# WeijingShi/Point-GNN

Hardware: AMD Instinct MI355X
Metric: KITTI-shaped frames/sec (car_auto_T3 inference: graph build + GNN, 20000 pts/frame, mean E1 602k) (higher is better)
Workload: dtype f32

## Files before the change

point-gnn_amd/csrc/edge_ws.h:

```cpp
#pragma once
#include "mlp_engine.h"
#include "ws_partition.h"

namespace pgnn {

#ifndef PGNN_WS_SCHED
#define PGNN_WS_SCHED 2
#endif

constexpr int kWsWaves = 8;
constexpr int kWsSchedInts = 2 + kWsMaxSlices * kWsMaxGroups;
constexpr int kWsStampTiles = 38;
constexpr int kWsStampStride = 8 + 4 * kWsStampTiles;

struct EdgeWsArgs {
  const float *P, *Q;
  int ldv4;
  const int32_t *edges;
  int64_t n_edges;
  const int32_t *n_dev;
  const float *wp;
  int nt;
  int relu_from;
  float *out;
  int64_t ldo;
  int num_segments;
  int sorted;
  int xcds;
  int prio;
  long long *ts;
  int32_t *sched;
  int pool_pct;
  int chunk;
  int groups;
  int tile0[kWsMaxGroups + 1];
  int wg0[kWsMaxGroups + 1];
  int balanced;
  int n_wg[kWsMaxGroups];
  short swg0[kWsMaxSlices][kWsMaxGroups + 1];
  short sbase[kWsMaxSlices][kWsMaxGroups];
  float *rows_out;
  int64_t ld_rows;
  float *h1_out;
  const int32_t *nv_dev;
};

__device__ __forceinline__ float opaque_inf() {
  float inf;
  asm("v_mov_b32 %0, 0x7f800000" : "=v"(inf));
  return inf;
}
__device__ __forceinline__ float max_nc(float a, float b, float inf) {
  return __builtin_amdgcn_fmed3f(a, b, inf);
}

typedef float v2f __attribute__((ext_vector_type(2)));
__device__ __forceinline__ v2f pk_sub(v2f a, v2f b) {
  v2f d;
  asm("v_pk_add_f32 %0, %1, %2 neg_lo:[0,1] neg_hi:[0,1]"
      : "=v"(d)
      : "v"(a), "v"(b));
  return d;
}

template <int CTRL>
__device__ __forceinline__ float dpp_mov(float x) {
  return __int_as_float(
      __builtin_amdgcn_update_dpp(0, __float_as_int(x), CTRL, 0xF, 0xF, false));
}

template <int NTG>
__device__ __forceinline__ float ws_v(const v4f (&v)[NTG], int i) {
  return i < 4 * NTG ? v[i >> 2][i & 3] : kFloatLowest;
}

template <int NTG, class ARGS>
__device__ __forceinline__ void ws_flush(const ARGS &a, const float *bias_lds,
                                         int t0, int lane, int d,
                                         const v4f (&v)[NTG], bool whole,
                                         float inf) {
  if (d < 0 || d >= a.num_segments) return;
  int zero;
  asm volatile("s_mov_b32 %0, 0" : "=s"(zero));
  const int n = (lane & 15) + zero, g = lane >> 4;
  const bool b0 = n & 1, b1 = n & 2, b2 = n & 4, b3 = n & 8;
  float A[16], B[8], C[4], D[2];
#pragma unroll
  for (int j = 0; j < 16; ++j) {
    if (2 * j < 4 * NTG) {
      const float x0 = ws_v<NTG>(v, 2 * j), x1 = ws_v<NTG>(v, 2 * j + 1);
      A[j] = max_nc(b0 ? x1 : x0, dpp_mov<0xB1>(b0 ? x0 : x1), inf);
    } else {
      A[j] = kFloatLowest;
    }
  }
#pragma unroll
  for (int k = 0; k < 8; ++k)
    B[k] = max_nc(b1 ? A[2 * k + 1] : A[2 * k],
                  dpp_mov<0x4E>(b1 ? A[2 * k] : A[2 * k + 1]), inf);
#pragma unroll
  for (int l = 0; l < 4; ++l)
    C[l] = max_nc(b2 ? B[2 * l + 1] : B[2 * l],
                  __shfl_xor(b2 ? B[2 * l] : B[2 * l + 1], 4), inf);
#pragma unroll
  for (int m = 0; m < 2; ++m)
    D[m] = max_nc(b3 ? C[2 * m + 1] : C[2 * m],
                  __shfl_xor(b3 ? C[2 * m] : C[2 * m + 1], 8), inf);
  float *orow = a.out + (int64_t)d * a.ldo + 16 * t0;
#pragma unroll
  for (int m = 0; m < 2; ++m) {
    const int i = 16 * m + n;
    if (i < 4 * NTG) {
      const int c = 16 * (i >> 2) + 4 * g + (i & 3);
      float x = D[m] + bias_lds[c];
      if (16 * t0 + c >= a.relu_from) x = x > 0.0f ? x : 0.0f;
      if (whole)
        orow[c] = x;
      else
        atomic_max_f32(orow + c, x + 0.0f);
    }
  }
}

struct WsRun {
  int cur_d;
  bool left_closed;
  bool has;
};

template <int NTG, class ARGS>
__device__ __forceinline__ void ws_epilogue(const ARGS &a, const float *bias_lds,
                                            int t0, int lane,
                                            const v4f (&acc)[NTG],
                                            v4f (&carry)[NTG], unsigned starts,
                                            int my_d, WsRun &st, bool fin,
                                            int d_after, float inf) {
  const int n = lane & 15;
  int cur_d = st.cur_d;
  bool cur_left_closed = st.left_closed, cur_has = st.has;
  int pos = 0;
  if (!(starts & 1u)) {
    const int f = starts ? __builtin_ctz(starts) : 16;
    if (f == 16) {
#pragma unroll
      for (int t = 0; t < NTG; ++t)
#pragma unroll
        for (int r = 0; r < 4; ++r)
          carry[t][r] = max_nc(carry[t][r], acc[t][r], inf);
    } else {
      const bool in_run = n < f;
#pragma unroll
      for (int t = 0; t < NTG; ++t)
#pragma unroll
        for (int r = 0; r < 4; ++r)
          carry[t][r] =
              max_nc(carry[t][r], in_run ? acc[t][r] : kFloatLowest, inf);
    }
    cur_has = true;
    pos = f;
  }
  while (pos < 16) {
    if (cur_has)
      ws_flush<NTG>(a, bias_lds, t0, lane, cur_d, carry,
                    a.sorted && cur_left_closed &&
                        (!fin || d_after != cur_d),
                    inf);
    if (fin) break;
    const unsigned rest = starts & ~((2u << pos) - 1u);
    const int nextpos = rest ? __builtin_ctz(rest) : 16;
    const bool in_run = n >= pos && n < nextpos;
#pragma unroll
    for (int t = 0; t < NTG; ++t)
#pragma unroll
      for (int r = 0; r < 4; ++r)
        carry[t][r] = in_run ? acc[t][r] : kFloatLowest;
    cur_d = __builtin_amdgcn_readlane(my_d, pos);
    cur_left_closed = true;
    cur_has = true;
    pos = nextpos;
  }
  st.cur_d = cur_d;
  st.left_closed = cur_left_closed;
  st.has = cur_has;
}

}

#include "ws_sum.h"

namespace pgnn {

template <int KQ, int NTG, bool EMIT, bool ROWS = false, class POL = WsMax>
__device__ __forceinline__ void edge_ws_body(const EdgeWsArgs &a,
                                             const v4f *__restrict__ wl, int t0,
                                             const float *bias_lds,
                                             int64_t tile_first,
                                             int64_t tile_last, int lane,
                                             long long *tsw, int &stamped,
                                             const int64_t E) {
  if (tile_first >= tile_last) return;
  const int n = lane & 15;
  const int64_t e_first = tile_first * 16;
  const int64_t e_end = tile_last * 16 < E ? tile_last * 16 : E;
  const v4f *__restrict__ P4 = reinterpret_cast<const v4f *>(a.P);
  const v4f *__restrict__ Q4 = reinterpret_cast<const v4f *>(a.Q);
  const int2 *__restrict__ e2 = reinterpret_cast<const int2 *>(a.edges);

// ... 390 lines not shown
```

point-gnn_amd/csrc/mlp_engine.h:

```cpp
#pragma once
#include "pgnn_common.h"

namespace pgnn {

#ifndef PGNN_PF4
#define PGNN_PF4 2
#endif
#ifndef PGNN_PF1
#define PGNN_PF1 4
#endif

typedef float v4f __attribute__((ext_vector_type(4)));

struct LayerDev {
  const float *wp;
  int kq;
  int nt;
  int relu_from;
};

struct ChainDev {
  int n;
  LayerDev l[PGNN_MAX_LAYERS];
};
// ... 339 lines not shown
#pragma unroll
      for (int r = 0; r < NR; ++r)
        accr[r] = __builtin_amdgcn_mfma_f32_16x16x4f32(fa_r[s], fb_r[r][s],
                                                       accr[r], 0, 0, 0);
    }
  };
#pragma unroll
  for (int st = 0; st < PF; ++st) fetch(st, a[st], b[st], ar[st], br[st]);
  for (int q = 0; q < kq; q += PF) {
#pragma unroll
    for (int st = 0; st < PF; ++st) {
      if (q + st < kq) {
        mma(a[st], b[st], ar[st], br[st], 0, 4);
        fetch(q + st + PF, a[st], b[st], ar[st], br[st]);
      }
    }
  }
}

__device__ __forceinline__ float activate(const LayerDev &L, const float *bias,
                                          int col, float x) {
  x += bias[col];
  if (col >= L.relu_from) x = x > 0.0f ? x : 0.0f;
  return x;
}

template <int NT, int NR, bool TRANSPOSED>
__device__ __forceinline__ void store_split(float *__restrict__ out, int ldo,
                                            const LayerDev &L, int t0, int wave,
                                            int lane, const v4f (&acc)[4][NT],
                                            const v4f (&accr)[NR]) {
  if (TRANSPOSED)
    store_acc_T<4, NT>(out, L, t0, wave, lane, acc);
  else
    store_acc<4, NT>(out, ldo, L, t0, wave, lane, acc);
  const float *bias = L.wp + (size_t)L.kq * L.nt * 256;
  constexpr int ROWS = 64, G = ROWS / 4, SWZ = 15;
#pragma unroll
  for (int r = 0; r < NR; ++r) {
    const int col = (t0 + 4 * NT + r) * 16 + (lane & 15);
    const int c = col - 16 * t0;
    v4f v;
#pragma unroll
    for (int i = 0; i < 4; ++i) v[i] = activate(L, bias, col, accr[r][i]);
    if (TRANSPOSED) {
      const int g = 4 * wave + (lane >> 4);
      *reinterpret_cast<v4f *>(out + c * ROWS + ((g ^ (c & SWZ)) << 2)) = v;
    } else {
      float *o = out + (16 * wave + 4 * (lane >> 4)) * ldo + c;
#pragma unroll
      for (int i = 0; i < 4; ++i) o[i * ldo] = v[i];
    }
  }
  (void)G;
}

template <int NT, int NR, bool TRANSPOSED>
__device__ __forceinline__ void layer_pass_split(const float *in, int ld_in,
                                                 float *out, int ld_out,
                                                 const LayerDev &L, int t0,
                                                 int wave, int lane) {
  v4f acc[4][NT], accr[NR];
  gemm_tile_split<NT, NR>(in, ld_in, L, t0, wave, lane, acc, accr);
  __syncthreads();
  store_split<NT, NR, TRANSPOSED>(out, ld_out, L, t0, wave, lane, acc, accr);
  __syncthreads();
}

__device__ __forceinline__ void lds_atomic_max_f32(float *addr, float v) {
  if (v >= 0.0f) {
    __hip_atomic_fetch_max((int *)addr, __float_as_int(v), __ATOMIC_RELAXED,
                           __HIP_MEMORY_SCOPE_WORKGROUP);
  } else {
    __hip_atomic_fetch_min((unsigned int *)addr, __float_as_uint(v),
                           __ATOMIC_RELAXED, __HIP_MEMORY_SCOPE_WORKGROUP);
  }
}

__device__ __forceinline__ void segfast_emit(const SegFast &sf, int col,
                                             float v) {
  if (sf.merge) v = fmaxf(v, sf.carry[col]);
  if (sf.defer) {
    sf.carry[col] = v;
  } else if (sf.whole) {
    sf.out_row[col] = v;
  } else {
    atomic_max_f32(sf.out_row + col, v + 0.0f);
  }
}

template <int NT, int NR>
__device__ __forceinline__ void layer_pass_segmax_fast_split(
    const float *in, int ld_in, const LayerDev &L, int t0, int wave, int lane,
    const SegFast &sf, float *part) {
  v4f acc[4][NT], accr[NR];
  gemm_tile_split<NT, NR>(in, ld_in, L, t0, wave, lane, acc, accr);
  const float *bias = L.wp + (size_t)L.kq * L.nt * 256;
#pragma unroll
  for (int r = 0; r < NR; ++r) {
    float v = fmaxf(fmaxf(accr[r][0], accr[r][1]),
                    fmaxf(accr[r][2], accr[r][3]));
    v = fmaxf(v, __shfl_xor(v, 16));
    v = fmaxf(v, __shfl_xor(v, 32));
    if (lane < 16) lds_atomic_max_f32(part + r * 16 + lane, v + 0.0f);
  }
#pragma unroll
  for (int j = 0; j < NT; ++j) {
    float v = acc[0][j][0];
#pragma unroll
    for (int m = 0; m < 4; ++m)
#pragma unroll
      for (int i = 0; i < 4; ++i) v = fmaxf(v, acc[m][j][i]);
    v = fmaxf(v, __shfl_xor(v, 16));
    v = fmaxf(v, __shfl_xor(v, 32));
    const int col = (t0 + wave + 4 * j) * 16 + (lane & 15);
    if (lane < 16) segfast_emit(sf, col, activate(L, bias, col, v));
  }
}

template <int NT, int NR>
__device__ __forceinline__ void segfast_finish_split(const LayerDev &L, int t0,
                                                     const SegFast &sf,
                                                     float *part) {
  if (threadIdx.x < 16 * NR) {
    const float *bias = L.wp + (size_t)L.kq * L.nt * 256;
    const int col = (t0 + 4 * NT) * 16 + threadIdx.x;
    const float v = part[threadIdx.x];
    part[threadIdx.x] = kFloatLowest;
    segfast_emit(sf, col, activate(L, bias, col, v));
  }
}

__device__ __forceinline__ bool use_split(int msub, int tiles) {
  return msub == 4 && tiles == 19;
}

template <int MSUB>
__device__ __forceinline__ bool layer_pass_segmax_fast_auto(
    const float *in, int ld_in, const LayerDev &L, int t0, int wave, int lane,
    const SegFast &sf, float *part) {
  int tiles = L.nt - t0;
  if (tiles > kMaxTilesPerPass) tiles = kMaxTilesPerPass;
  if constexpr (MSUB == 4) {
    if (use_split(MSUB, tiles)) {
      layer_pass_segmax_fast_split<4, 3>(in, ld_in, L, t0, wave, lane, sf,
                                         part);
      return true;
    }
  }
  layer_pass_segmax_fast_dispatch<MSUB>(in, ld_in, L, t0, wave, lane, sf);
  return false;
}

template <int KQ, int NT, int TBMAX = 8>
__device__ __forceinline__ void reg_layer(const LayerDev &L, int lane,
                                          const v4f (&in)[KQ], v4f (&out)[NT]) {
  int zero;
  asm volatile("s_mov_b32 %0, 0" : "=s"(zero));
  const v4f *__restrict__ wp =
      reinterpret_cast<const v4f *>(L.wp) + lane + zero;
  const float *bias = L.wp + (size_t)KQ * NT * 256 + zero;
  const int g4 = 4 * (lane >> 4) + zero;
  constexpr int TB = NT < TBMAX ? NT : TBMAX;
  static_assert(NT % TB == 0, "column tiles come in blocks");
#pragma unroll
  for (int t0 = 0; t0 < NT; t0 += TB) {
    v4f w[2][TB];
#pragma unroll
    for (int j = 0; j < TB; ++j) {
      out[t0 + j] = (v4f){0.f, 0.f, 0.f, 0.f};
      w[0][j] = wp[(size_t)(t0 + j) * 64];
    }
#pragma unroll
    for (int q = 0; q < KQ; ++q) {
      if (q + 1 < KQ) {
#pragma unroll
        for (int j = 0; j < TB; ++j)
          w[(q + 1) & 1][j] = wp[((size_t)(q + 1) * NT + t0 + j) * 64];
      }
#pragma unroll
      for (int s = 0; s < 4; ++s)
#pragma unroll
        for (int j = 0; j < TB; ++j)
          out[t0 + j] = __builtin_amdgcn_mfma_f32_16x16x4f32(
              w[q & 1][j][s], in[q][s], out[t0 + j], 0, 0, 0);
      __builtin_amdgcn_sched_barrier(0);
    }
#pragma unroll
    for (int j = 0; j < TB; ++j) {
      const int t = t0 + j;
      const v4f b = *reinterpret_cast<const v4f *>(bias + 16 * t + g4);
#pragma unroll
      for (int r = 0; r < 4; ++r) {
        float v = out[t][r] + b[r];
        if (16 * t + g4 + r >= L.relu_from) v = v > 0.0f ? v : 0.0f;
        out[t][r] = v;
      }
    }
  }
}

template <int KQ, int... NTS>
struct RegChain;

template <int KQ>
struct RegChain<KQ> {
  static __device__ __forceinline__ void run(const ChainDev &, int, int lane,
                                             const v4f (&in)[KQ],
                                             float *__restrict__ rows16,
                                             int ld) {
    float *o = rows16 + (lane & 15) * ld + 4 * (lane >> 4);
#pragma unroll
    for (int q = 0; q < KQ; ++q) *reinterpret_cast<v4f *>(o + 16 * q) = in[q];
  }
};

template <int KQ, int NT, int... REST>
struct RegChain<KQ, NT, REST...> {
  static __device__ __forceinline__ void run(const ChainDev &chain, int li,
                                             int lane, const v4f (&in)[KQ],
                                             float *__restrict__ rows16,
                                             int ld) {
    v4f out[NT];
    reg_layer<KQ, NT>(chain.l[li], lane, in, out);
    RegChain<NT, REST...>::run(chain, li + 1, lane, out, rows16, ld);
  }
};

template <int MSUB, int NT, bool TRANSPOSED, int NW = 4>
__device__ __forceinline__ void layer_pass(const float *in, int ld_in, float *out,
                                           int ld_out, const LayerDev &L, int t0,
                                           int wave, int lane, bool skip_gemm) {
  static_assert(!TRANSPOSED || NW == 4, "transposed stage is 4-wave only");
  v4f acc[MSUB][NT];
  if (!skip_gemm) {
    gemm_tile<MSUB, NT, NW>(in, ld_in, L, t0, wave, lane, acc);
  } else {
#pragma unroll
    for (int m = 0; m < MSUB; ++m)
#pragma unroll
      for (int j = 0; j < NT; ++j) acc[m][j] = (v4f){0.f, 0.f, 0.f, 0.f};
  }
  __syncthreads();
  if constexpr (TRANSPOSED)
    store_acc_T<MSUB, NT>(out, L, t0, wave, lane, acc);
  else
    store_acc<MSUB, NT, NW>(out, ld_out, L, t0, wave, lane, acc);
  __syncthreads();
}

constexpr int kKrowNT = 3;

template <int PF>
struct KrowPreT {
  v4f b[PF][kKrowNT];
  float bias[kKrowNT];
};
using KrowPre = KrowPreT<PGNN_PF1>;

template <int PF>
__device__ __forceinline__ void krow_prefetch_w(const LayerDev &L, int t0,
                                                int wave, int lane,
                                                KrowPreT<PF> &p) {
  const v4f *__restrict__ wp = reinterpret_cast<const v4f *>(L.wp) + lane;
  const int qstride = L.nt * 64;
#pragma unroll
  for (int j = 0; j < kKrowNT; ++j) {
    int t = t0 + wave + 8 * j;
    if (t > L.nt - 1) t = L.nt - 1;
#pragma unroll
    for (int st = 0; st < PF; ++st) {
      const int q = st < L.kq ? st : L.kq - 1;
      p.b[st][j] = wp[(size_t)q * qstride + t * 64];
    }
  }
}

template <int PF>
__device__ __forceinline__ void krow_prefetch_bias(const LayerDev &L, int t0,
                                                   int wave, int lane,
                                                   KrowPreT<PF> &p) {
  const float *__restrict__ bias = L.wp + (size_t)L.kq * L.nt * 256;
#pragma unroll
  for (int j = 0; j < kKrowNT; ++j) {
    int t = t0 + wave + 8 * j;
    if (t > L.nt - 1) t = L.nt - 1;
    p.bias[j] = bias[t * 16 + (lane & 15)];
  }
}

template <int PF>
__device__ __forceinline__ void krow_prefetch(const LayerDev &L, int t0, int wave,
                                              int lane, KrowPreT<PF> &p) {
  krow_prefetch_w(L, t0, wave, lane, p);
  krow_prefetch_bias(L, t0, wave, lane, p);
}

template <int NT, int PF>
__device__ __forceinline__ void krow_gemm(const float *in, int ld_in,
                                          const LayerDev &L, int t0, int wave,
                                          int lane, KrowPreT<PF> &pre,
                                          v4f (&acc)[kKrowNT]) {
  constexpr int NW = 8;
  static_assert(NT <= kKrowNT, "prefetch slots");
  if constexpr (NT > 0) {
  int toff[NT];
#pragma unroll
  for (int j = 0; j < NT; ++j) {
    acc[j] = (v4f){0.f, 0.f, 0.f, 0.f};
    int t = t0 + wave + NW * j;
    if (t > L.nt - 1) t = L.nt - 1;
    toff[j] = t * 64;
  }
  const v4f *__restrict__ wp = reinterpret_cast<const v4f *>(L.wp) + lane;
  const float *arow = in + (lane & 15) * ld_in + 4 * (lane >> 4);
  const int qstride = L.nt * 64;
  const int kq = L.kq;
  v4f a[PF];
#pragma unroll
  for (int st = 0; st < PF; ++st)
    a[st] = *reinterpret_cast<const v4f *>(arow + 16 * (st < kq ? st : kq - 1));
  int q = 0;
  for (; q + PF <= kq; q += PF) {
#pragma unroll
    for (int st = 0; st < PF; ++st) {
#pragma unroll
      for (int s = 0; s < 4; ++s)
#pragma unroll
        for (int j = 0; j < NT; ++j)
          acc[j] = __builtin_amdgcn_mfma_f32_16x16x4f32(
              a[st][s], pre.b[st][j][s], acc[j], 0, 0, 0);
      int qn = q + st + PF;
      if (qn > kq - 1) qn = kq - 1;
#pragma unroll
      for (int j = 0; j < NT; ++j)
        pre.b[st][j] = wp[(size_t)qn * qstride + toff[j]];
      a[st] = *reinterpret_cast<const v4f *>(arow + 16 * qn);
    }
  }
  const int rem = kq - q;
#pragma unroll
  for (int st = 0; st + 1 < PF; ++st) {
    if (st < rem) {
#pragma unroll
      for (int s = 0; s < 4; ++s)
#pragma unroll
        for (int j = 0; j < NT; ++j)
          acc[j] = __builtin_amdgcn_mfma_f32_16x16x4f32(
              a[st][s], pre.b[st][j][s], acc[j], 0, 0, 0);
    }
  }
  }
// ... 68 lines not shown
```

point-gnn_amd/csrc/pool_split.h:

```cpp
#pragma once
#include "pool_ws.h"

namespace pgnn {

__device__ __forceinline__ void pool_hidden_body(const PoolWsArgs &a,
                                                 const v4f *__restrict__ wl,
                                                 const float *bias_lds,
                                                 int64_t tile_first,
                                                 int64_t tile_last, int lane,
                                                 const int64_t E) {
  constexpr int KQ = 8, NT = 16, NTB = 8;
  if (tile_first >= tile_last) return;
  const int n = lane & 15;
  const int64_t e_first = tile_first * 16;
  const int2 *__restrict__ e2 = reinterpret_cast<const int2 *>(a.edges);
  bool nxt_ok = e_first + n < E;
  int2 nxt = e2[nxt_ok ? e_first + n : 0];
  int nxt_k;
  {
    const int d0 = nxt_ok ? nxt.y : 0;
    nxt_k = a.kp[((unsigned)d0 < (unsigned)a.num_segments) ? d0 : 0];
  }
  for (int64_t tile = tile_first; tile < tile_last; ++tile) {
    const int64_t e0 = tile * 16;
    if (a.prio) __builtin_amdgcn_s_setprio(3);
    int lz;
    asm volatile("v_mov_b32 %0, %1" : "=v"(lz) : "v"(lane));
    const int g = lz >> 4;
    int lz1 = lz + 64 * 64, lz2 = lz + 128 * 64;
    asm volatile("" : "+v"(lz1));
    asm volatile("" : "+v"(lz2));
    const v4f *const wfrag[3] = {wl + lz, wl + lz1, wl + lz2};
    const bool ok = nxt_ok;
    const int my_s = ok ? nxt.x : 0;
    const int my_k = nxt_k;
    nxt_ok = tile + 1 < tile_last && e0 + 16 + n < E;
    nxt = e2[nxt_ok ? e0 + 16 + n : 0];
    v4f x[1];
    x[0] = (v4f){0.f, 0.f, 0.f, 0.f};
    if (ok) {
#pragma unroll
      for (int i = 0; i < 4; ++i) {
        const int c = 4 * g + i;
        float v = 0.0f;
        if (c < a.nfeat) {
          v = a.feat[(int64_t)my_s * a.nfeat + c];
        } else if (c < a.nfeat + 3) {
          const int ax = c - a.nfeat;
          v = a.xyz[3 * (int64_t)my_s + ax] - a.xyz[3 * (int64_t)my_k + ax];
        }
        x[0][i] = v;
      }
    }
    __builtin_amdgcn_sched_barrier(0);
    __builtin_amdgcn_s_setprio(0);
    v4f h1[2], h2[4], h3[KQ];
#ifdef PGNN_POOL_ABL_NO_HIDDEN
#pragma unroll
    for (int q = 0; q < KQ; ++q) h3[q] = x[0];
#else
    reg_layer<1, 2>(a.l0, lane, x, h1);
    reg_layer<2, 4>(a.l1, lane, h1, h2);
    reg_layer<4, 8>(a.l2, lane, h2, h3);
#endif
    __builtin_amdgcn_sched_barrier(0);
    {
      const int dn = nxt_ok ? nxt.y : 0;
      nxt_k = a.kp[((unsigned)dn < (unsigned)a.num_segments) ? dn : 0];
    }
#pragma unroll
    for (int tb = 0; tb < NT; tb += NTB) {
      v4f acc[NTB];
      pool_ws_block<KQ, NT, NTB>(wfrag, tb, h3, acc);
      if (e0 + n < E) {
        float *dstp = a.a4_out + (e0 + n) * a.ld4 + 16 * tb + 4 * g;
#pragma unroll
        for (int t = 0; t < NTB; ++t) {
          const v4f bb =
              *reinterpret_cast<const v4f *>(bias_lds + 16 * (tb + t) + 4 * g);
          v4f y;
#pragma unroll
          for (int r = 0; r < 4; ++r) {
            float xx = acc[t][r] + bb[r];
            if (16 * (tb + t) + 4 * g + r >= a.relu_from)
              xx = xx > 0.0f ? xx : 0.0f;
            y[r] = xx;
          }
          *reinterpret_cast<v4f *>(dstp + 16 * t) = y;
        }
      }
    }
  }
  __builtin_amdgcn_s_setprio(0);
}

#ifndef PGNN_POOLH_WAVES
#define PGNN_POOLH_WAVES 12
#endif
constexpr int kPoolHWaves = PGNN_POOLH_WAVES;
__global__ __launch_bounds__(64 * kPoolHWaves) void pool_hidden_kernel(PoolWsArgs a) {
  constexpr int KQ = 8, NT = 16;
  constexpr int kWsWaves = kPoolHWaves;
  extern __shared__ __attribute__((aligned(16))) char smem[];
  v4f *wl = reinterpret_cast<v4f *>(smem);
  float *bias_lds = reinterpret_cast<float *>(wl + KQ * NT * 64);
  const int lane = threadIdx.x & 63;
  const int wave = __builtin_amdgcn_readfirstlane(threadIdx.x >> 6);
  {
    const v4f *__restrict__ src = reinterpret_cast<const v4f *>(a.wp);
    constexpr int PER = (KQ * NT + kWsWaves - 1) / kWsWaves;
    v4f tmp[PER];
#pragma unroll
    for (int i = 0; i < PER; ++i) {
      const int f = wave + i * kWsWaves;
      tmp[i] = src[(size_t)(f < KQ * NT ? f : 0) * 64 + lane];
    }
    __builtin_amdgcn_sched_barrier(0);
#pragma unroll
    for (int i = 0; i < PER; ++i) {
      const int f = wave + i * kWsWaves;
      if (f < KQ * NT) wl[(size_t)f * 64 + lane] = tmp[i];
    }
    if ((int)threadIdx.x < 16 * NT)
      bias_lds[threadIdx.x] = a.wp[(size_t)KQ * NT * 256 + threadIdx.x];
  }
  __syncthreads();
  int64_t n_edges = a.n_edges;
  if (a.n_dev) {
    const int64_t nd = *a.n_dev;
    n_edges = nd < n_edges ? nd : n_edges;
  }
  const int64_t n_wt = (n_edges + 15) / 16;
  const int xcds = a.slices;
  const int slice = blockIdx.x % xcds, local = blockIdx.x / xcds;
  const int64_t s_first = n_wt * slice / xcds;
  const int64_t s_last = n_wt * (slice + 1) / xcds;
  const int64_t nw = (int64_t)(gridDim.x / xcds) * kWsWaves;
  const int64_t wi = (int64_t)local * kWsWaves + wave;
  const int64_t span = s_last - s_first;
  pool_hidden_body(a, wl, bias_lds, s_first + span * wi / nw,
                   s_first + span * (wi + 1) / nw, lane, n_edges);
}

}
```

point-gnn_amd/csrc/pool_ws.h:

```cpp
#pragma once
#include "edge_ws.h"

namespace pgnn {

struct PoolWsArgs {
  const float *feat;
  int nfeat;
  const float *xyz;
  const int32_t *kp;
  const int32_t *edges;
  int64_t n_edges;
  const int32_t *n_dev;
  LayerDev l0, l1, l2;
  const float *wp;
  int kq, nt;
  int relu_from;
  float *out;
  int64_t ldo;
  int num_segments;
  int sorted;
  int prio;
  long long *ts;
  int32_t *sched;
  int pool_pct;
  int chunk;
  int slices;
  float *a1_out, *a2_out, *a3_out, *a4_out;
  int64_t ld4;
  const void *l2_f16;
};

__device__ __forceinline__ int pool_kp_of(const PoolWsArgs &a, bool ok, int2 e) {
  const int d = ok ? e.y : 0;
  return a.kp[((unsigned)d < (unsigned)a.num_segments) ? d : 0];
}

template <int KQ, int NT, int NTB>
__device__ __forceinline__ void pool_ws_block(const v4f *const (&wfrag)[3],
                                              int tb, const v4f (&h)[KQ],
                                              v4f (&acc)[NTB]) {
  v4f w[2][NTB];
#pragma unroll
  for (int t = 0; t < NTB; ++t) {
    acc[t] = (v4f){0.f, 0.f, 0.f, 0.f};
    w[0][t] = wfrag[(tb + t) >> 6][((tb + t) & 63) * 64];
  }
  __builtin_amdgcn_sched_barrier(0);
#pragma unroll
  for (int q = 0; q < KQ; ++q) {
    __builtin_amdgcn_s_waitcnt(0xC07F);
    __builtin_amdgcn_sched_barrier(0);
    if (q + 1 < KQ) {
#pragma unroll
      for (int t = 0; t < NTB; ++t)
        w[(q + 1) & 1][t] = wfrag[((q + 1) * NT + tb + t) >> 6]
                                 [(((q + 1) * NT + tb + t) & 63) * 64];
    }
#pragma unroll
    for (int s = 0; s < 4; ++s)
#pragma unroll
      for (int t = 0; t < NTB; ++t)
        acc[t] = __builtin_amdgcn_mfma_f32_16x16x4f32(w[q & 1][t][s], h[q][s],
                                                      acc[t], 0, 0, 0);
#if PGNN_WS_SCHED == 2
#pragma unroll
    for (int t = 0; t < NTB; ++t) {
      __builtin_amdgcn_sched_group_barrier(0x8 , 3, 0);
      if (q + 1 < KQ)
        __builtin_amdgcn_sched_group_barrier(0x100 , 1, 0);
    }
    __builtin_amdgcn_sched_group_barrier(0x8 , NTB, 0);
#else
    if (q + 1 < KQ)
      __builtin_amdgcn_sched_group_barrier(0x100 , NTB, 0);
    __builtin_amdgcn_sched_group_barrier(0x8 , 4 * NTB, 0);
#endif
    __builtin_amdgcn_sched_barrier(0);
  }
}

template <bool EMIT, class POL = WsMax>
__device__ __forceinline__ void pool_ws_body(const PoolWsArgs &a,
                                             const v4f *__restrict__ wl,
                                             const float *bias_lds,
                                             int64_t tile_first,
                                             int64_t tile_last, int lane,
                                             long long *tsw, int &stamped,
                                             const int64_t E) {
  constexpr int KQ = 8, NT = 19;
  if (tile_first >= tile_last) return;
  const int n = lane & 15;
  const int64_t e_first = tile_first * 16;
  const int64_t e_end = tile_last * 16 < E ? tile_last * 16 : E;
  const int2 *__restrict__ e2 = reinterpret_cast<const int2 *>(a.edges);
  int cur_d = e_first > 0 ? a.edges[2 * (e_first - 1) + 1] : -1;
  int d_after = e_end < E ? a.edges[2 * e_end + 1] : -1;
  cur_d = __builtin_amdgcn_readfirstlane(cur_d);
  d_after = __builtin_amdgcn_readfirstlane(d_after);
  WsRun run = {cur_d, false, false};
  constexpr float kIdentity = POL::kSum ? 0.0f : kFloatLowest;
  v4f carry0[7], carry1[6], carry2[6];
#pragma unroll
  for (int t = 0; t < 7; ++t) {
    carry0[t] = (v4f){kIdentity, kIdentity, kIdentity, kIdentity};
    if (t < 6) {
      carry1[t] = (v4f){kIdentity, kIdentity, kIdentity, kIdentity};
      carry2[t] = (v4f){kIdentity, kIdentity, kIdentity, kIdentity};
    }
  }
  const float inf = opaque_inf();
  bool nxt_ok = e_first + n < E;
  int2 nxt = e2[nxt_ok ? e_first + n : 0];
  int nxt_k = pool_kp_of(a, nxt_ok, nxt);
  for (int64_t tile = tile_first;; ++tile) {
    const bool fin = tile >= tile_last;
    const int64_t e0 = tile * 16;
    if (a.prio) __builtin_amdgcn_s_setprio(3);
    int lz;
    asm volatile("v_mov_b32 %0, %1" : "=v"(lz) : "v"(lane));
    const int g = lz >> 4;
    int lz1 = lz + 64 * 64, lz2 = lz + 128 * 64;
    asm volatile("" : "+v"(lz1));
    asm volatile("" : "+v"(lz2));
    const v4f *const wfrag[3] = {wl + lz, wl + lz1, wl + lz2};
    long long *tst = nullptr;
    if (tsw && !fin && stamped < kWsStampTiles) tst = tsw + 8 + 4 * stamped++;
    if (tst) {
      __builtin_amdgcn_sched_barrier(0);
      const long long c = __builtin_readcyclecounter();
      if (lane == 0) tst[0] = c;
      __builtin_amdgcn_sched_barrier(0);
    }
    unsigned starts = 1u;
    int my_d = -1;
    v4f h3[KQ];
    if (fin) {
#pragma unroll
      for (int q = 0; q < KQ; ++q) h3[q] = (v4f){0.f, 0.f, 0.f, 0.f};
    } else {
      const bool ok = nxt_ok;
      const int my_s = ok ? nxt.x : 0;
      my_d = ok ? nxt.y : -1;
      const int my_k = nxt_k;
      nxt_ok = tile + 1 < tile_last && e0 + 16 + n < E;
      nxt = e2[nxt_ok ? e0 + 16 + n : 0];
      v4f x[1];
      x[0] = (v4f){0.f, 0.f, 0.f, 0.f};
      if (ok) {
#pragma unroll
        for (int i = 0; i < 4; ++i) {
          const int c = 4 * g + i;
          float v = 0.0f;
          if (c < a.nfeat) {
            v = a.feat[(int64_t)my_s * a.nfeat + c];
          } else if (c < a.nfeat + 3) {
            const int ax = c - a.nfeat;
            v = a.xyz[3 * (int64_t)my_s + ax] - a.xyz[3 * (int64_t)my_k + ax];
          }
          x[0][i] = v;
        }
      }
      __builtin_amdgcn_sched_barrier(0);
      if (tst) {
        const long long c = __builtin_readcyclecounter();
        if (lane == 0) tst[1] = c;
        __builtin_amdgcn_sched_barrier(0);
      }
      __builtin_amdgcn_s_setprio(0);
      v4f h1[2], h2[4];
#ifdef PGNN_POOL_ABL_NO_HIDDEN
#pragma unroll
      for (int q = 0; q < KQ; ++q) h3[q] = x[0];
      h1[0] = h1[1] = x[0];
#pragma unroll
      for (int q = 0; q < 4; ++q) h2[q] = x[0];
#else
      reg_layer<1, 2>(a.l0, lane, x, h1);
      reg_layer<2, 4>(a.l1, lane, h1, h2);
      reg_layer<4, 8>(a.l2, lane, h2, h3);
#endif
      if constexpr (EMIT) {
        if (e0 + n < E) {
          const int64_t row = e0 + n;
#pragma unroll
          for (int q = 0; q < 2; ++q)
            *reinterpret_cast<v4f *>(a.a1_out + row * 32 + 16 * q + 4 * g) = h1[q];
#pragma unroll
          for (int q = 0; q < 4; ++q)
            *reinterpret_cast<v4f *>(a.a2_out + row * 64 + 16 * q + 4 * g) = h2[q];
#pragma unroll
          for (int q = 0; q < 8; ++q)
            *reinterpret_cast<v4f *>(a.a3_out + row * 128 + 16 * q + 4 * g) = h3[q];
        }
      }
      __builtin_amdgcn_sched_barrier(0);
      nxt_k = pool_kp_of(a, nxt_ok, nxt);
      const int up = __shfl_up(my_d, 1);
      const int prev = n == 0 ? run.cur_d : up;
      starts = (unsigned)(__ballot(my_d != prev) & 0xFFFFull);
    }
    const WsRun run0 = run;
#define PGNN_POOL_WS_BLOCK(NTB, TB, CARRY)                                     \
    {                                                                          \
      v4f acc[NTB];                                                            \
      if (!fin) {                                                              \
        pool_ws_block<KQ, NT, NTB>(wfrag, TB, h3, acc);                        \
        if constexpr (EMIT) {     \
          if (e0 + n < E) {                                                    \
            float *dstp = a.a4_out + (e0 + n) * a.ld4 + 16 * (TB) + 4 * g;     \
            _Pragma("unroll")                                                  \
            for (int t = 0; t < NTB; ++t) {                                    \
              const v4f bb = *reinterpret_cast<const v4f *>(                   \
                  bias_lds + 16 * ((TB) + t) + 4 * g);                         \
              v4f y;                                                           \
              _Pragma("unroll")                                                \
              for (int r = 0; r < 4; ++r) {                                    \
                float xx = acc[t][r] + bb[r];                                  \
                if (16 * ((TB) + t) + 4 * g + r >= a.relu_from)                \
                  xx = xx > 0.0f ? xx : 0.0f;                                  \
                y[r] = xx;                                                     \
              }                                                                \
              *reinterpret_cast<v4f *>(dstp + 16 * t) = y;                     \
            }                                                                  \
          }                                                                    \
        }                                                                      \
      } else {       \
        _Pragma("unroll")        \
        for (int t = 0; t < NTB; ++t) acc[t] = (v4f){0.f, 0.f, 0.f, 0.f};      \
      }                                                                        \
      if (a.prio) __builtin_amdgcn_s_setprio(3);                               \
      run = run0;                                                              \
      if constexpr (POL::kSum)                                                 \
        ws_epilogue_sum<NTB>(a, bias_lds + 16 * (TB), TB, lane, acc, CARRY,    \
                             starts, my_d, run, fin, d_after, inf);            \
      else                                                                     \
        ws_epilogue<NTB>(a, bias_lds + 16 * (TB), TB, lane, acc, CARRY,        \
                         starts, my_d, run, fin, d_after, inf);                \
      __builtin_amdgcn_s_setprio(0);                                           \
    }
    PGNN_POOL_WS_BLOCK(7, 0, carry0)
    PGNN_POOL_WS_BLOCK(6, 7, carry1)
    PGNN_POOL_WS_BLOCK(6, 13, carry2)
#undef PGNN_POOL_WS_BLOCK
    if (fin) break;
    if (tst) {
      __builtin_amdgcn_sched_barrier(0);
      const long long c = __builtin_readcyclecounter();
      if (lane == 0) {
        tst[2] = c;
        tst[3] = c;
      }
    }
  }
  __builtin_amdgcn_s_setprio(0);
}

template <bool EMIT = false, class POL = WsMax>
__global__ __launch_bounds__(64 * kWsWaves) void pool_ws_kernel(PoolWsArgs a) {
  constexpr int KQ = 8, NT = 19;
  extern __shared__ __attribute__((aligned(16))) char smem[];
  v4f *wl = reinterpret_cast<v4f *>(smem);
  float *bias_lds = reinterpret_cast<float *>(wl + KQ * NT * 64);
  const int lane = threadIdx.x & 63;
  const int wave = __builtin_amdgcn_readfirstlane(threadIdx.x >> 6);
  ws_stage<(KQ * NT + kWsWaves - 1) / kWsWaves>(
      a, wl, KQ * NT, [](int f) { return (size_t)f; }, (size_t)KQ * NT * 256,
      0, NT, bias_lds, wave, lane);
  __syncthreads();
  const int64_t n_edges = ws_edge_count(a.n_edges, a.n_dev);
  const int64_t n_wt = (n_edges + 15) / 16;
  const int64_t nw = (int64_t)gridDim.x * kWsWaves;
  const int64_t wi = (int64_t)blockIdx.x * kWsWaves + wave;
  const int64_t pool = ws_pool_size(n_wt, a.sched, a.pool_pct, 2, nw);
  const int64_t span = n_wt - pool;
  int64_t tile_first = span * wi / nw;
  int64_t tile_last = span * (wi + 1) / nw;
  long long *tsw = nullptr;
  if (a.ts) {
    tsw = a.ts + wi * kWsStampStride;
    if (lane == 0) {
      tsw[0] = __builtin_readcyclecounter();
      tsw[2] = __builtin_amdgcn_s_memrealtime();
      tsw[4] = tile_last - tile_first;
      tsw[5] = NT;
      tsw[6] = 0;
    }
  }
  int stamped = 0;
  for (;;) {
    pool_ws_body<EMIT, POL>(a, wl, bias_lds, tile_first, tile_last, lane, tsw,
                       stamped, n_edges);
    if (pool == 0) break;
    const int c = ws_pool_claim(&a.sched[2], a.chunk, lane);
    if (c >= pool) break;
    tile_first = span + c;
    tile_last = tile_first + a.chunk < n_wt ? tile_first + a.chunk : n_wt;
  }
  if (tsw && lane == 0) {
    tsw[1] = __builtin_readcyclecounter();
    tsw[3] = __builtin_amdgcn_s_memrealtime();
    tsw[7] = stamped;
  }
  ws_pool_rearm(a.sched, 1, lane);
}

}
```

point-gnn_amd/csrc/ws_launch.h:

```cpp
#pragma once
#include "ws_partition.h"

namespace {
using namespace pgnn;

inline int ws_cus(int cus) {
  return (g_ws_reserve > 0 && cus - g_ws_reserve >= 64) ? cus - g_ws_reserve : cus;
}
inline int ws_cus(hipStream_t stream) { return ws_cus(stream_cu_count(stream)); }

inline int ws_slices(int cus) { return ws_slice_count(cus, g_ws_xcds); }
inline bool ws_feasible(int nt, int ntmax, int cus) {
  return pgnn::ws_feasible(nt, ntmax, cus, ws_slices(cus));
}

inline int ws_partition_rc(int why) {
  PGNN_REQUIRE(why != kWsTooFewCus, PGNN_E_UNSUPPORTED,
               "edge_ws: too few CUs for the column groups");
  PGNN_REQUIRE(why == kWsOk, PGNN_E_UNSUPPORTED,
               "edge_ws: column tiles do not group");
  return 0;
}

template <int KQ, int NTMAX>
int plan_edge_ws(EdgeWsArgs &a, const LayerDev &L, const EdgeArgs &ea,
                 int64_t n_edges, const SegArgs &sa, int cus, int32_t *sched,
                 float *rows_out, int64_t ld_rows, float *h1_out,
                 const int32_t *n_dev) {
  a = {};
  const int rc = ws_partition_rc(ws_partition(a, L.nt, NTMAX, cus, ws_slices(cus)));
  if (rc) return rc;
  a.n_dev = n_dev;
  a.rows_out = rows_out;
  a.ld_rows = ld_rows;
  a.h1_out = h1_out;
  a.P = ea.P;
  a.Q = ea.Q;
  a.ldv4 = (int)(ea.ldpq >> 2);
  a.edges = ea.edges;
  a.n_edges = n_edges;
  a.wp = L.wp;
  a.nt = L.nt;
  a.relu_from = L.relu_from;
  a.out = sa.out;
  a.ldo = sa.ldo;
  a.num_segments = sa.num_segments;
  a.sorted = sa.sorted;
  a.prio = g_ws_prio;
  a.ts = (long long *)g_mlp_ts;
  a.sched = (g_ws_pool_pct > 0 && a.xcds <= kWsMaxSlices) ? sched : nullptr;
  a.pool_pct = g_ws_pool_pct;
  a.chunk = g_ws_chunk;
  if (g_ws_balance >= 2) {
    double cost[kWsMaxGroups];
    for (int g = 0; g < a.groups; ++g)
      cost[g] = 128.0 * KQ * (a.tile0[g + 1] - a.tile0[g]) + 1900.0;
    ws_balance(a, cus, cost, a.sched != nullptr);
  }
  return 0;
}

template <int KQ, int NTMAX, bool ROWS, class POL = WsMax>
int run_edge_ws(const EdgeWsArgs &a, int cus, hipStream_t stream) {
  static_assert(!POL::kSum || !ROWS, "the sum kernels read no ready rows");
  PGNN_HIP((hipError_t)arm_sched(a.sched, stream));
  const size_t lds = (size_t)KQ * NTMAX * 1024 + 16 * NTMAX * sizeof(float);
  auto kern = edge_ws_kernel<KQ, NTMAX, false, ROWS, POL>;
  if constexpr (!ROWS && !POL::kSum) {
    if (a.rows_out) kern = edge_ws_kernel<KQ, NTMAX, true>;
  }
  return launch_lds(kern, dim3((unsigned)(cus / a.xcds * a.xcds)),
                    dim3(64 * kWsWaves), lds, stream, a);
}

template <int KQ, int NTMAX, class POL = WsMax>
int launch_edge_ws(const LayerDev &L, const EdgeArgs &ea, int64_t n_edges,
                   const SegArgs &sa, int cus, int32_t *sched,
                   hipStream_t stream, float *rows_out = nullptr,
                   int64_t ld_rows = 0, float *h1_out = nullptr,
                   const int32_t *n_dev = nullptr) {
  EdgeWsArgs a;
  const int rc = plan_edge_ws<KQ, NTMAX>(a, L, ea, n_edges, sa, cus, sched,
                                         rows_out, ld_rows, h1_out, n_dev);
  return rc ? rc : run_edge_ws<KQ, NTMAX, false, POL>(a, cus, stream);
}

template <class POL = WsMax>
bool edge_ws_applies(const Plan &p, int64_t n_edges, int cus) {
  if (g_mlp_debug & 2048) return false;
  const LayerDev &L = p.chain.l[0];
  if (p.chain.n != 1 || L.kq != L.nt || (L.nt != 19 && L.nt != 16)) return false;
  if (cus < 64 || cus % 8 != 0) return false;
  if (!ws_feasible(L.nt, L.nt == 19 ? 7 : 8, cus)) return false;
  if ((size_t)L.kq * (L.nt == 19 ? 7 : 8) * 1024 + 16 * 8 * sizeof(float) >
      device_max_lds())
    return false;
  if (g_mlp_debug & 4096) return true;
  return n_edges >= (int64_t)16 * 2 * kWsWaves * cus;
}

template <class POL = WsMax>
bool pool_ws_applies(const Plan &p, int64_t n_edges, int cus) {
  if (g_mlp_debug & (8192 | 1024)) return false;
  const ChainDev &c = p.chain;
  if (c.n != 4 || c.l[0].kq != 1 || c.l[0].nt != 2 || c.l[1].nt != 4 ||
      c.l[2].nt != 8 || c.l[3].kq != 8 || c.l[3].nt != 19)
    return false;
  if (cus < 8) return false;
  if ((size_t)8 * 19 * 1024 + 16 * 19 * sizeof(float) > device_max_lds())
    return false;
  if (g_mlp_debug & 16384) return true;
  return n_edges >= (int64_t)16 * 2 * kWsWaves * cus;
}

PoolWsArgs pool_ws_args(const Plan &p, const PoolArgs &pa, int64_t n_edges,
                        const int32_t *n_dev, int num_segments) {
  PoolWsArgs a = {};
  a.feat = pa.feat;
  a.nfeat = pa.nfeat;
  a.xyz = pa.xyz;
  a.kp = pa.kp;
  a.edges = pa.edges;
  a.n_edges = n_edges;
  a.n_dev = n_dev;
  a.l0 = p.chain.l[0];
  a.l1 = p.chain.l[1];
  a.l2 = p.chain.l[2];
  a.wp = p.chain.l[3].wp;
  a.kq = p.chain.l[3].kq;
  a.nt = p.chain.l[3].nt;
  a.relu_from = p.chain.l[3].relu_from;
  a.num_segments = num_segments;
  return a;
}

int pool_ws_out(PoolWsArgs &a, const SegArgs &sa, int32_t *sched,
                hipStream_t stream) {
  a.out = sa.out;
  a.ldo = sa.ldo;
  a.sorted = sa.sorted;
  a.sched = g_ws_pool_pct > 0 ? sched : nullptr;
  a.pool_pct = g_ws_pool_pct;
  a.chunk = 1;
  PGNN_HIP((hipError_t)arm_sched(a.sched, stream));
  return 0;
}

template <class POL = WsMax>
int launch_pool_ws(const Plan &p, const PoolArgs &pa, int64_t n_edges,
                   const SegArgs &sa, int cus, int32_t *sched,
                   hipStream_t stream, float *const *acts = nullptr,
                   int64_t ld4 = 0, const int32_t *n_dev = nullptr) {
  PoolWsArgs a = pool_ws_args(p, pa, n_edges, n_dev, sa.num_segments);
  if (acts) {
    a.a1_out = acts[0];
    a.a2_out = acts[1];
    a.a3_out = acts[2];
    a.a4_out = acts[3];
    a.ld4 = ld4;
  }
  a.prio = g_ws_prio;
  a.ts = (long long *)g_mlp_ts;
  const int rc = pool_ws_out(a, sa, sched, stream);
  if (rc) return rc;
  const size_t lds = (size_t)8 * 19 * 1024 + 16 * 19 * sizeof(float);
  auto kern = pool_ws_kernel<false, POL>;
  if constexpr (!POL::kSum) {
    if (acts) kern = pool_ws_kernel<true>;
  }
  return launch_lds(kern, dim3((unsigned)cus), dim3(64 * kWsWaves), lds, stream,
                    a);
}

constexpr int kPoolSplitHidden = 256;
bool pool_split_applies(const Plan &p, int64_t n_edges, int cus) {
  if (g_mlp_debug & (8192 | 1024)) return false;
  const ChainDev &c = p.chain;
  if (c.n != 5 || c.l[0].kq != 1 || c.l[0].nt != 2 || c.l[1].nt != 4 ||
      c.l[2].nt != 8 || c.l[3].kq != 8 || c.l[3].nt != 16 || c.l[4].kq != 16 ||
      c.l[4].nt != 32)
    return false;
  if (cus < 64 || cus % 8 != 0) return false;
  if (!ws_feasible(c.l[4].nt, 8, cus)) return false;
  if ((size_t)16 * 8 * 1024 + 16 * 16 * sizeof(float) > device_max_lds())
    return false;
  if (g_mlp_debug & 16384) return true;
  return n_edges >= (int64_t)16 * 2 * kWsWaves * cus;
}

int launch_pool_split(const Plan &p, const PoolArgs &pa, int64_t n_edges,
                      const SegArgs &sa, int cus, int32_t *sched,
                      hipStream_t stream, const int32_t *n_dev, float *hidden) {
  const EdgeArgs ea = {hidden, nullptr, kPoolSplitHidden, pa.edges};
  EdgeWsArgs e;
  int rc = plan_edge_ws<16, 8>(e, p.chain.l[4], ea, n_edges, sa, cus, sched,
                               nullptr, 0, nullptr, n_dev);
  if (rc) return rc;
  PoolWsArgs a = pool_ws_args(p, pa, n_edges, n_dev, sa.num_segments);
  a.prio = g_ws_prio;
  a.a4_out = hidden;
  a.ld4 = kPoolSplitHidden;
  a.slices = 8;
  const size_t lds = (size_t)8 * 16 * 1024 + 16 * 16 * sizeof(float);
  rc = launch_lds(pool_hidden_kernel, dim3((unsigned)cus),
                  dim3(64 * kPoolHWaves), lds, stream, a);
  return rc ? rc : run_edge_ws<16, 8, true>(e, cus, stream);
}

template <class Arith>
struct SplitHost;
template <>
struct SplitHost<Bf16x3> {
  static constexpr const char *kName = "edge_bf16x3";
  static constexpr int kNtMax10 = 5, kNtMax8 = 5;
  static constexpr double kTileCost = 960.0, kRowCost = 2400.0;
  static int prio() { return g_ws_prio; }
};
template <>
struct SplitHost<F16x2> {
  static constexpr const char *kName = "edge_f16x2";
  static constexpr int kNtMax10 = 7, kNtMax8 = 6;
  static constexpr double kTileCost = 480.0, kRowCost = 1600.0;
  static int prio() { return 0; }
};

template <class Arith>
std::string split_msg(const char *what) {
  return std::string(SplitHost<Arith>::kName) + ": " + what;
}

template <class Arith, int KB, int NTMAX>
int launch_edge_ws_split(EdgeWsArgs &a, int nt, int cus, int32_t *status,
                         hipStream_t stream) {
  using H = SplitHost<Arith>;
  const int rc = ws_partition_rc(ws_partition(a, nt, NTMAX, cus, ws_slices(cus)));
  if (rc) return rc;
  if (g_ws_balance) {
    double cost[kWsMaxGroups];
    for (int g = 0; g < a.groups; ++g)
      cost[g] = H::kTileCost * KB / 10 * (a.tile0[g + 1] - a.tile0[g]) + H::kRowCost;
    ws_balance(a, cus, cost, a.sched != nullptr);
  }
  const size_t lds =
      (size_t)KB * NTMAX * Arith::kParts * 1024 + 16 * NTMAX * sizeof(float);
  PGNN_REQUIRE(lds <= device_max_lds(), PGNN_E_UNSUPPORTED,
               split_msg<Arith>("column group does not fit the LDS").c_str());
  return launch_lds(edge_ws_split_kernel<Arith, KB, NTMAX>,
                    dim3((unsigned)(cus / a.xcds * a.xcds)), dim3(64 * kWsWaves),
                    lds, stream, a, status);
}

template <class Arith>
int edge_split_fwd_impl(const float *P, const float *Q, int64_t ld_pq,
                        int32_t width, const int32_t *edges, int64_t edges_cap,
                        int32_t vertices_cap, const void *image, int32_t n_out,
                        int32_t relu_from, int32_t edges_sorted, float *out,
                        int64_t ld_out, int32_t *status,
                        const pgnn_dyn_count *n_edges,
                        const pgnn_dyn_count *num_vertices, hipStream_t stream) {
  using H = SplitHost<Arith>;
  PGNN_REQUIRE(edges_cap >= 0 && vertices_cap >= 0 && width > 0 && n_out > 0 &&
                   image,
               PGNN_E_INVALID, split_msg<Arith>("bad argument").c_str());
  const Dyn de = dyn_of(n_edges), dk = dyn_of(num_vertices);
  const int kq = (width + 15) / 16, nt = (n_out + 15) / 16;
  const int kb = (width + 31) / 32;
  PGNN_REQUIRE(ld_pq == 16 * kq && ld_out >= 16 * nt, PGNN_E_INVALID,
               split_msg<Arith>("ld_pq / ld_out do not match the padded widths")
                   .c_str());
  const int cus = ws_cus(stream);
  if (!((kb == 10 && nt == 19) || (kb == 8 && nt == 16)) || cus < 64 ||
      cus % 8 != 0 ||
      !ws_feasible(nt, kb == 10 ? H::kNtMax10 : H::kNtMax8, cus) ||
      (!g_b16_force &&
       expected(de, edges_cap) < (int64_t)16 * 2 * kWsWaves * cus) ||
      (int64_t)vertices_cap * ld_pq * 4 >= ((int64_t)1 << 32))
    return PGNN_E_UNSUPPORTED;
  if (vertices_cap == 0) return 0;
  PGNN_REQUIRE(out != nullptr, PGNN_E_INVALID,
               split_msg<Arith>("null output").c_str());
  if (!(edges_sorted & 2)) {
    const int rc = fill_lowest_rows(out, ld_out, vertices_cap, dk, stream);
    if (rc) return rc;
  }
  if (edges_cap == 0) return 0;
  PGNN_REQUIRE(P && Q && edges, PGNN_E_INVALID,
               split_msg<Arith>("null input").c_str());
  PGNN_REQUIRE(((uintptr_t)P % 16 == 0) && ((uintptr_t)Q % 16 == 0) &&
                   ((uintptr_t)image % 16 == 0),
               PGNN_E_INVALID,
               split_msg<Arith>("P / Q / image must be 16-byte aligned").c_str());
  EdgeWsArgs a = {};
  a.P = P;
  a.Q = Q;
  a.ldv4 = (int)(ld_pq >> 2);
  a.edges = edges;
  a.n_edges = edges_cap;
  a.n_dev = de.dev;
  a.wp = reinterpret_cast<const float *>(image);
  a.nt = nt;
  a.relu_from = relu_from;
  a.out = out;
  a.ldo = ld_out;
  a.num_segments = vertices_cap;
  a.sorted = edges_sorted & 1;
  a.prio = H::prio();
  if (Arith::kRangeGuard) a.nv_dev = dk.dev;
  if (kb == 10)
    return launch_edge_ws_split<Arith, 10, H::kNtMax10>(a, nt, cus, status, stream);
  return launch_edge_ws_split<Arith, 8, H::kNtMax8>(a, nt, cus, status, stream);
}

}
```

Before: 326.6.

## Pipeline hidden-layer weight fetches across layers and stage hidden biases in LDS

Splits the register MLP layer into fetch and run stages so the next layer's first weight fragments are loaded during the previous layer's MFMA work, with sched_group_barrier interleaving loads and MFMAs. The pool_ws kernel also stages the hidden-layer biases and the first layer's weights in LDS, and uses a branch-free fmed3 ReLU when every column is rectified. The aim is to hide global-load latency in the small per-tile hidden MLP, at the cost of more live VGPRs and a slightly larger LDS footprint, which could lower occupancy.

```diff
diff --git a/point-gnn_amd/csrc/edge_ws.h b/point-gnn_amd/csrc/edge_ws.h
--- a/point-gnn_amd/csrc/edge_ws.h
+++ b/point-gnn_amd/csrc/edge_ws.h
@@ -45,14 +45,6 @@
   const int32_t *nv_dev;
 };
 
-__device__ __forceinline__ float opaque_inf() {
-  float inf;
-  asm("v_mov_b32 %0, 0x7f800000" : "=v"(inf));
-  return inf;
-}
-__device__ __forceinline__ float max_nc(float a, float b, float inf) {
-  return __builtin_amdgcn_fmed3f(a, b, inf);
-}
 
 typedef float v2f __attribute__((ext_vector_type(2)));
 __device__ __forceinline__ v2f pk_sub(v2f a, v2f b) {
diff --git a/point-gnn_amd/csrc/mlp_engine.h b/point-gnn_amd/csrc/mlp_engine.h
--- a/point-gnn_amd/csrc/mlp_engine.h
+++ b/point-gnn_amd/csrc/mlp_engine.h
@@ -515,52 +515,119 @@
   return false;
 }
 
-template <int KQ, int NT, int TBMAX = 8>
+__device__ __forceinline__ float opaque_inf() {
+  float inf;
+  asm("v_mov_b32 %0, 0x7f800000" : "=v"(inf));
+  return inf;
+}
+__device__ __forceinline__ float max_nc(float a, float b, float inf) {
+  return __builtin_amdgcn_fmed3f(a, b, inf);
+}
+
+struct RegSrc {
+  const v4f *w;
+  const float *bias;
+  int g4;
+  int relu_from;
+};
+
+__device__ __forceinline__ int reg_opaque_zero() {
+  int zero;
+  asm volatile("s_mov_b32 %0, 0" : "=s"(zero));
+  return zero;
+}
+
+template <int KQ, int NT>
+__device__ __forceinline__ RegSrc reg_src(const LayerDev &L, int lane,
+                                          const v4f *w_frags,
+                                          const float *bias) {
+  const int zero = reg_opaque_zero();
+  RegSrc s;
+  s.w = w_frags + lane + zero;
+  s.g4 = 4 * (lane >> 4) + zero;
+  s.bias = bias + s.g4;
+  s.relu_from = L.relu_from;
+  return s;
+}
+template <int KQ, int NT>
+__device__ __forceinline__ const float *reg_bias_of(const LayerDev &L) {
+  return L.wp + (size_t)KQ * NT * 256;
+}
+template <int KQ, int NT>
+__device__ __forceinline__ RegSrc reg_src(const LayerDev &L, int lane) {
+  return reg_src<KQ, NT>(L, lane, reinterpret_cast<const v4f *>(L.wp),
+                         reg_bias_of<KQ, NT>(L));
+}
+
+template <int NT>
+__device__ __forceinline__ void reg_fetch0(const RegSrc &S, v4f (&w0)[NT]) {
+#pragma unroll
+  for (int j = 0; j < NT; ++j) w0[j] = S.w[(size_t)j * 64];
+}
+
+template <int KQ, int NT, class NEXT>
+__device__ __forceinline__ void reg_layer_run(const RegSrc &S, float inf,
+                                              const v4f (&in)[KQ],
+                                              v4f (&w0)[NT], v4f (&out)[NT],
+                                              NEXT &&next) {
+  static_assert(NT <= 8, "two stages of weight fragments: 8 NT VGPRs");
+  v4f w1[NT], b[NT];
+#pragma unroll
+  for (int j = 0; j < NT; ++j) out[j] = (v4f){0.f, 0.f, 0.f, 0.f};
+#pragma unroll
+  for (int q = 0; q < KQ; ++q) {
+    v4f(&cur)[NT] = (q & 1) ? w1 : w0;
+    v4f(&nxt)[NT] = (q & 1) ? w0 : w1;
+    if (q + 1 < KQ) {
+#pragma unroll
+      for (int j = 0; j < NT; ++j)
+        nxt[j] = S.w[((size_t)(q + 1) * NT + j) * 64];
+    } else {
+#pragma unroll
+      for (int j = 0; j < NT; ++j)
+        b[j] = *reinterpret_cast<const v4f *>(S.bias + 16 * j);
+    }
+#pragma unroll
+    for (int s = 0; s < 4; ++s)
+#pragma unroll
+      for (int j = 0; j < NT; ++j)
+        out[j] = __builtin_amdgcn_mfma_f32_16x16x4f32(cur[j][s], in[q][s],
+                                                      out[j], 0, 0, 0);
+    __builtin_amdgcn_sched_group_barrier(0x20 , NT, 0);
+    __builtin_amdgcn_sched_group_barrier(0x100 , NT, 0);
+    __builtin_amdgcn_sched_group_barrier(0x8 , 4 * NT, 0);
+    __builtin_amdgcn_sched_barrier(0);
+  }
+  next();
+  __builtin_amdgcn_sched_barrier(0);
+#ifndef PGNN_REG_EPILOGUE_GENERAL
+#define PGNN_REG_EPILOGUE_GENERAL 0
+#endif
+  if (!PGNN_REG_EPILOGUE_GENERAL && S.relu_from <= 0) {
+#pragma unroll
+    for (int j = 0; j < NT; ++j)
+#pragma unroll
+      for (int r = 0; r < 4; ++r)
+        out[j][r] = max_nc(out[j][r] + b[j][r], 0.0f, inf);
+  } else {
+#pragma unroll
+    for (int j = 0; j < NT; ++j)
+#pragma unroll
+      for (int r = 0; r < 4; ++r) {
+        float v = out[j][r] + b[j][r];
+        if (16 * j + S.g4 + r >= S.relu_from) v = v > 0.0f ? v : 0.0f;
+        out[j][r] = v;
+      }
+  }
+}
+
+template <int KQ, int NT>
 __device__ __forceinline__ void reg_layer(const LayerDev &L, int lane,
                                           const v4f (&in)[KQ], v4f (&out)[NT]) {
-  int zero;
-  asm volatile("s_mov_b32 %0, 0" : "=s"(zero));
-  const v4f *__restrict__ wp =
-      reinterpret_cast<const v4f *>(L.wp) + lane + zero;
-  const float *bias = L.wp + (size_t)KQ * NT * 256 + zero;
-  const int g4 = 4 * (lane >> 4) + zero;
-  constexpr int TB = NT < TBMAX ? NT : TBMAX;
-  static_assert(NT % TB == 0, "column tiles come in blocks");
-#pragma unroll
-  for (int t0 = 0; t0 < NT; t0 += TB) {
-    v4f w[2][TB];
-#pragma unroll
-    for (int j = 0; j < TB; ++j) {
-      out[t0 + j] = (v4f){0.f, 0.f, 0.f, 0.f};
-      w[0][j] = wp[(size_t)(t0 + j) * 64];
-    }
-#pragma unroll
-    for (int q = 0; q < KQ; ++q) {
-      if (q + 1 < KQ) {
-#pragma unroll
-        for (int j = 0; j < TB; ++j)
-          w[(q + 1) & 1][j] = wp[((size_t)(q + 1) * NT + t0 + j) * 64];
-      }
-#pragma unroll
-      for (int s = 0; s < 4; ++s)
-#pragma unroll
-        for (int j = 0; j < TB; ++j)
-          out[t0 + j] = __builtin_amdgcn_mfma_f32_16x16x4f32(
-              w[q & 1][j][s], in[q][s], out[t0 + j], 0, 0, 0);
-      __builtin_amdgcn_sched_barrier(0);
-    }
-#pragma unroll
-    for (int j = 0; j < TB; ++j) {
-      const int t = t0 + j;
-      const v4f b = *reinterpret_cast<const v4f *>(bias + 16 * t + g4);
-#pragma unroll
-      for (int r = 0; r < 4; ++r) {
-        float v = out[t][r] + b[r];
-        if (16 * t + g4 + r >= L.relu_from) v = v > 0.0f ? v : 0.0f;
-        out[t][r] = v;
-      }
-    }
-  }
+  const RegSrc S = reg_src<KQ, NT>(L, lane);
+  v4f w0[NT];
+  reg_fetch0<NT>(S, w0);
+  reg_layer_run<KQ, NT>(S, opaque_inf(), in, w0, out, [] {});
 }
 
 template <int KQ, int... NTS>
diff --git a/point-gnn_amd/csrc/pool_split.h b/point-gnn_amd/csrc/pool_split.h
--- a/point-gnn_amd/csrc/pool_split.h
+++ b/point-gnn_amd/csrc/pool_split.h
@@ -14,6 +14,7 @@
   const int n = lane & 15;
   const int64_t e_first = tile_first * 16;
   const int2 *__restrict__ e2 = reinterpret_cast<const int2 *>(a.edges);
+  const float inf = opaque_inf();
   bool nxt_ok = e_first + n < E;
   int2 nxt = e2[nxt_ok ? e_first + n : 0];
   int nxt_k;
@@ -36,6 +37,12 @@
     const int my_k = nxt_k;
     nxt_ok = tile + 1 < tile_last && e0 + 16 + n < E;
     nxt = e2[nxt_ok ? e0 + 16 + n : 0];
+    const RegSrc s0 = reg_src<1, 2>(a.l0, lane);
+    const RegSrc s1 = reg_src<2, 4>(a.l1, lane);
+    const RegSrc s2 = reg_src<4, 8>(a.l2, lane);
+    v4f w0[2], w1[4], w2[8];
+    reg_fetch0<2>(s0, w0);
+    reg_fetch0<4>(s1, w1);
     v4f x[1];
     x[0] = (v4f){0.f, 0.f, 0.f, 0.f};
     if (ok) {
@@ -59,9 +66,9 @@
 #pragma unroll
     for (int q = 0; q < KQ; ++q) h3[q] = x[0];
 #else
-    reg_layer<1, 2>(a.l0, lane, x, h1);
-    reg_layer<2, 4>(a.l1, lane, h1, h2);
-    reg_layer<4, 8>(a.l2, lane, h2, h3);
+    reg_layer_run<1, 2>(s0, inf, x, w0, h1, [] {});
+    reg_layer_run<2, 4>(s1, inf, h1, w1, h2, [&] { reg_fetch0<8>(s2, w2); });
+    reg_layer_run<4, 8>(s2, inf, h2, w2, h3, [] {});
 #endif
     __builtin_amdgcn_sched_barrier(0);
     {
diff --git a/point-gnn_amd/csrc/pool_ws.h b/point-gnn_amd/csrc/pool_ws.h
--- a/point-gnn_amd/csrc/pool_ws.h
+++ b/point-gnn_amd/csrc/pool_ws.h
@@ -83,6 +83,8 @@
 __device__ __forceinline__ void pool_ws_body(const PoolWsArgs &a,
                                              const v4f *__restrict__ wl,
                                              const float *bias_lds,
+                                             const float *hid_bias_lds,
+                                             const v4f *w0_lds,
                                              int64_t tile_first,
                                              int64_t tile_last, int lane,
                                              long long *tsw, int &stamped,
@@ -144,6 +146,13 @@
       const int my_k = nxt_k;
       nxt_ok = tile + 1 < tile_last && e0 + 16 + n < E;
       nxt = e2[nxt_ok ? e0 + 16 + n : 0];
+      const RegSrc s0 = reg_src<1, 2>(a.l0, lane, w0_lds, hid_bias_lds);
+      const RegSrc s1 = reg_src<2, 4>(
+          a.l1, lane, reinterpret_cast<const v4f *>(a.l1.wp), hid_bias_lds + 32);
+      const RegSrc s2 = reg_src<4, 8>(
+          a.l2, lane, reinterpret_cast<const v4f *>(a.l2.wp), hid_bias_lds + 96);
+      v4f w0[2], w1[4], w2[8];
+      reg_fetch0<4>(s1, w1);
       v4f x[1];
       x[0] = (v4f){0.f, 0.f, 0.f, 0.f};
       if (ok) {
@@ -175,9 +184,10 @@
 #pragma unroll
       for (int q = 0; q < 4; ++q) h2[q] = x[0];
 #else
-      reg_layer<1, 2>(a.l0, lane, x, h1);
-      reg_layer<2, 4>(a.l1, lane, h1, h2);
-      reg_layer<4, 8>(a.l2, lane, h2, h3);
+      reg_fetch0<2>(s0, w0);
+      reg_layer_run<1, 2>(s0, inf, x, w0, h1, [] {});
+      reg_layer_run<2, 4>(s1, inf, h1, w1, h2, [&] { reg_fetch0<8>(s2, w2); });
+      reg_layer_run<4, 8>(s2, inf, h2, w2, h3, [] {});
 #endif
       if constexpr (EMIT) {
         if (e0 + n < E) {
@@ -255,6 +265,10 @@
   __builtin_amdgcn_s_setprio(0);
 }
 
+constexpr size_t kPoolWsHidBias = 32 + 64 + 128;
+constexpr size_t kPoolWsLds = (size_t)8 * 19 * 1024 + 16 * 19 * sizeof(float) +
+                              kPoolWsHidBias * sizeof(float) + 2 * 1024;
+
 template <bool EMIT = false, class POL = WsMax>
 __global__ __launch_bounds__(64 * kWsWaves) void pool_ws_kernel(PoolWsArgs a) {
   constexpr int KQ = 8, NT = 19;
@@ -266,6 +280,19 @@
   ws_stage<(KQ * NT + kWsWaves - 1) / kWsWaves>(
       a, wl, KQ * NT, [](int f) { return (size_t)f; }, (size_t)KQ * NT * 256,
       0, NT, bias_lds, wave, lane);
+  float *hid_bias_lds = bias_lds + 16 * NT;
+  v4f *w0_lds = reinterpret_cast<v4f *>(hid_bias_lds + kPoolWsHidBias);
+  {
+    const int i = threadIdx.x;
+    if (i < 32)
+      hid_bias_lds[i] = a.l0.wp[1 * 2 * 256 + i];
+    else if (i < 96)
+      hid_bias_lds[i] = a.l1.wp[2 * 4 * 256 + i - 32];
+    else if (i < (int)kPoolWsHidBias)
+      hid_bias_lds[i] = a.l2.wp[4 * 8 * 256 + i - 96];
+    float *w0f = reinterpret_cast<float *>(w0_lds);
+    for (int f = i; f < 2 * 256; f += 64 * kWsWaves) w0f[f] = a.l0.wp[f];
+  }
   __syncthreads();
   const int64_t n_edges = ws_edge_count(a.n_edges, a.n_dev);
   const int64_t n_wt = (n_edges + 15) / 16;
@@ -288,8 +315,8 @@
   }
   int stamped = 0;
   for (;;) {
-    pool_ws_body<EMIT, POL>(a, wl, bias_lds, tile_first, tile_last, lane, tsw,
-                       stamped, n_edges);
+    pool_ws_body<EMIT, POL>(a, wl, bias_lds, hid_bias_lds, w0_lds, tile_first,
+                            tile_last, lane, tsw, stamped, n_edges);
     if (pool == 0) break;
     const int c = ws_pool_claim(&a.sched[2], a.chunk, lane);
     if (c >= pool) break;
diff --git a/point-gnn_amd/csrc/ws_launch.h b/point-gnn_amd/csrc/ws_launch.h
--- a/point-gnn_amd/csrc/ws_launch.h
+++ b/point-gnn_amd/csrc/ws_launch.h
@@ -107,8 +107,7 @@
       c.l[2].nt != 8 || c.l[3].kq != 8 || c.l[3].nt != 19)
     return false;
   if (cus < 8) return false;
-  if ((size_t)8 * 19 * 1024 + 16 * 19 * sizeof(float) > device_max_lds())
-    return false;
+  if (kPoolWsLds > device_max_lds()) return false;
   if (g_mlp_debug & 16384) return true;
   return n_edges >= (int64_t)16 * 2 * kWsWaves * cus;
 }
@@ -163,7 +162,7 @@
   a.ts = (long long *)g_mlp_ts;
   const int rc = pool_ws_out(a, sa, sched, stream);
   if (rc) return rc;
-  const size_t lds = (size_t)8 * 19 * 1024 + 16 * 19 * sizeof(float);
+  const size_t lds = kPoolWsLds;
   auto kern = pool_ws_kernel<false, POL>;
   if constexpr (!POL::kSum) {
     if (acts) kern = pool_ws_kernel<true>;
```

After: 327.3 (median of 6 runs). Within noise of the previous version (+0.2%).
